# adeebkor/fenicsx-fus

Measured on AMD Instinct MI355X. Metric: DOF-updates/sec (RK4 step) at p=4 hex fp64, higher is better.
Workload: dtype f64; 1 GPU; 3D homogeneous wave, hex p=4 f64, Linear RK4, weak scaling: 64^3 cells per GPU (BASELINE.json configs[1]); ndofs_global=16974593, cells_per_gpu=262144, medium=water, partition=x-slabs x1, transport=none, blocks=8192, mfma_contractions=False, mfma_4x4x4_index1=False, packed_fp32=False, lds_bytes_per_block=72504

## Files before the change

### fenicsx-fus_amd/csrc/fusmi.hip

```cpp
#include "../../include/fusmi.h"

#include <dlfcn.h>
#include <hip/hip_runtime.h>
#include <rccl/rccl.h>
#include <limits>

#include <algorithm>
#include <cmath>
#include <cstdio>
#include <cstring>
#include <atomic>
#include <map>
#include <mutex>
#include <tuple>
#include <memory>
#include <string>
#include <vector>

#include "kernels.hpp"
#include "layout.hpp"
#include "tables.hpp"

using namespace fus;

// ... 131 lines not shown

struct fus_op
{
  fus_ctx* ctx;
  int P, N, Nd, dtype;
  int tdim = 3;
  size_t ts;
  int64_t ncells, ndofs, nnodes;
  Layout L;
  std::vector<double> nodes, wts, D;
  std::vector<char> h_geom_x;
  std::vector<int32_t> h_geom_dm;
  int geom_order = 1, geom_nv = 8;
  std::vector<int32_t> h_dofmap;
  BlockArgs A{};
  std::vector<void*> allocs;
  int32_t *d_cell_perm = nullptr, *d_dof_perm = nullptr;
  int64_t *d_sh_ptr = nullptr, *d_sh_pairs = nullptr;
  void *d_G = nullptr, *d_detJ = nullptr, *d_Dg = nullptr, *d_partial = nullptr;
  void *d_tmp_x = nullptr, *d_tmp_b = nullptr, *d_tmp_c = nullptr, *d_tmp_coef = nullptr;
  size_t lds_bytes = 0;
  int deterministic = 0;
  int nfields = 1;
  bool affine = false;
  bool trilinear = false;
  bool mfma = false;
  bool ortho_mesh = false;
  bool diag = false;
  bool pk = false;
  void* d_Gc = nullptr;
// ... 8 lines not shown

struct fus_model
{
  fus_ctx* ctx;
  fus_op* op;
  int kind;
  hipGraphExec_t gexec = nullptr;
  int64_t gsteps = 0;
  double freq, amp, speed;
  void *u0 = nullptr, *v0 = nullptr, *u_ = nullptr, *v_ = nullptr, *un = nullptr, *vn = nullptr,
       *b = nullptr, *minv = nullptr, *m = nullptr, *coef = nullptr, *coef2 = nullptr;
  void* d_bsrc2 = nullptr;
  void* mn1 = nullptr;
  int64_t nb = 0, nb_int = 0;
  int32_t* d_bidx = nullptr;
  int32_t* d_blk_bnd_off = nullptr;
  int32_t *d_sh_ptr32 = nullptr, *d_sh_pairs32 = nullptr;
  uint64_t* d_bnd_mask = nullptr;
  int32_t* d_bnd_base = nullptr;
  void *d_bsrc = nullptr, *d_babs = nullptr;
  std::vector<void*> allocs;
  bool initialised = false;
  bool setup_done = false;
  int rk_order = 4;
  int forms = 0;
  int lean_rk4 = 1;
  bool bnd_valid = false;
  double bnd_tn = 0.0;
  int64_t rc_n = 0;
  int32_t* d_rc_idx = nullptr;
  void *d_rc_bas = nullptr, *d_rc_out = nullptr, *d_rec = nullptr;
// ... 65 lines not shown
};

template <typename T, int P, int OP, int ATOMIC, int STAGE, int NF, int GEOM, int TD = 3, int MF = 0, int PK = 0>
static int launch_block_op_v(fus_op* op, const T* geo, const T* coef, const T* x, T* bvec,
                             const StageArgs<T>& S, int blk_begin, int blk_count)
{
  if (blk_count <= 0)
    return FUS_OK;
  constexpr int N = P + 1;
  KArgs<T, N> K;
  for (int i = 0; i < N * N; ++i)
    K.Dk.d[i] = (T)op->D[i], K.Dk.dt[i] = (T)op->D[(i % N) * N + i / N];

  for (int i = 0; i < N; ++i)
    K.Dk.w[i] = (T)op->wts[i], K.Dk.x[i] = (T)op->nodes[i];
  static std::atomic<uint64_t> attr_set{0};
  const uint64_t dev_bit = 1ull << (op->ctx->device & 63);
  if (!(attr_set.load(std::memory_order_relaxed) & dev_bit))
  {
    HIPCHK(hipFuncSetAttribute(reinterpret_cast<const void*>(&k_block_op<T, P, OP, ATOMIC, STAGE, NF, GEOM, TD, MF, PK>),
                               hipFuncAttributeMaxDynamicSharedMemorySize, 160 * 1024));
    attr_set.fetch_or(dev_bit, std::memory_order_relaxed);
  }
  K.A = op->A;
  if (GEOM == GEOM_DIAG)
  {
    for (int q = 0; q < N; ++q)
      for (int i = 0; i < N; ++i)
      {
        double acc = 0;
        for (int m = 0; m < N; ++m)
          acc += op->D[m * N + q] * op->wts[m] * op->D[m * N + i];
        K.Dk.d[q * N + i] = K.Dk.dt[q * N + i] = (T)acc;
      }
  }
  K.A.blk_begin = blk_begin;
  K.A.blk_count = blk_count;
  K.Dg = static_cast<const T*>(op->d_Dg), K.geo = geo, K.coef = coef, K.x = x, K.bvec = bvec;
  K.partial = static_cast<T*>(op->d_partial);
  K.S = S;
  int grid = blk_count;
  if (GEOM != GEOM_STREAM && TD == 3 && op->ctx->walk != 0)
  {
    int per_cu = op->ctx->walk;
    if (per_cu < 0)
    {
      static std::mutex occ_mu;
      static std::map<std::tuple<int, int, size_t>, int> occ_cache;
      int occ = 0;
      {
        std::lock_guard<std::mutex> lk(occ_mu);
        const auto key = std::make_tuple(op->ctx->device, op->L.waves, op->lds_bytes);
        auto it = occ_cache.find(key);
        if (it == occ_cache.end())
        {
          int nb = 0;
          HIPCHK(hipOccupancyMaxActiveBlocksPerMultiprocessor(
              &nb, reinterpret_cast<const void*>(&k_block_op<T, P, OP, ATOMIC, STAGE, NF, GEOM, TD, MF, PK>), 64 * op->L.waves,
              op->lds_bytes));
          it = occ_cache.emplace(key, std::max(nb, 1)).first;
        }
        occ = it->second;
      }
      per_cu = (blk_count >= 4 * occ * op->ctx->num_cus) ? occ : 0;
    }
    if (per_cu > 0)
      grid = std::min(blk_count, per_cu * op->ctx->num_cus);
  }
  hipLaunchKernelGGL((k_block_op<T, P, OP, ATOMIC, STAGE, NF, GEOM, TD, MF, PK>), dim3(grid),
                     dim3(64 * op->L.waves), op->lds_bytes, op->ctx->stream, K);
  HIPCHK(hipGetLastError());
  return FUS_OK;
}

template <typename T, int P, int OP, int STAGE, int NF = 1>
static int launch_block_op(fus_op* op, const T* geo, const T* coef, const T* x, T* bvec,
                           const StageArgs<T>& S, int blk_begin = 0, int blk_count = -1)
{
  if (NF > op->nfields)
    return fail(FUS_ERR_STATE, "operator data was not created for two-field models (option fields=2)");
  if (blk_count < 0)
    blk_count = op->L.nblocks - blk_begin;
  const int b0 = blk_begin, nb = blk_count;
  if constexpr (P >= 8)
// ... 225 lines not shown
static bool mfma_default(int P, bool f64, bool affine)
{
  (void)P, (void)f64, (void)affine;
  return false;
}

template <typename T, int P>
static int op_setup_device(fus_op* op)
{
  constexpr int N = P + 1;
  fus_ctx* c = op->ctx;
  hipStream_t st = c->stream;
  Layout& L = op->L;
  auto& pool = op->allocs;

  std::vector<ShapeDev> shapes(L.shapes.size());
  for (size_t i = 0; i < shapes.size(); ++i)
  {
    shapes[i].nelem = L.shapes[i].nelem, shapes[i].nloc = L.shapes[i].nloc;
    shapes[i].nint = L.shapes[i].nint, shapes[i].nrounds = L.shapes[i].nrounds;
    shapes[i].rounds_off = L.shapes[i].rounds_off, shapes[i].ldm_off = L.shapes[i].ldm_off;
  }
  int32_t *d_blk_shape, *d_elem_off, *d_int_off, *d_sh_gidx;
  int64_t* d_sh_off;
  ShapeDev* d_shapes;
  int16_t* d_rounds;
  uint16_t* d_ldm;
  FUSCHK(upload(pool, &d_blk_shape, L.blk_shape, st));
  FUSCHK(upload(pool, &d_shapes, shapes, st));
  FUSCHK(upload(pool, &d_elem_off, L.blk_elem_off, st));
  FUSCHK(upload(pool, &d_int_off, L.blk_int_off, st));
  FUSCHK(upload(pool, &d_sh_off, L.blk_sh_off, st));
  FUSCHK(upload(pool, &d_sh_gidx, L.sh_gidx, st));
  FUSCHK(upload(pool, &d_rounds, L.rounds, st));
  L.ldm.resize((L.ldm.size() + 15) & ~(size_t)15);
  FUSCHK(upload(pool, &d_ldm, L.ldm, st));
  FUSCHK(upload(pool, &op->d_cell_perm, L.cell_perm, st));
  FUSCHK(upload(pool, &op->d_dof_perm, L.dof_perm, st));
  FUSCHK(upload(pool, &op->d_sh_ptr, L.sh_ptr, st));
  {
    std::vector<int64_t> pos(L.sh_pairs.size());
    for (size_t k = 0; k < pos.size(); ++k)
      pos[k] = L.pair_pos[L.sh_pairs[k]];
    FUSCHK(upload(pool, &op->d_sh_pairs, pos, st));
  }
  int32_t* d_sh_ppos;
  FUSCHK(upload(pool, &d_sh_ppos, L.pair_pos, st));
  op->A.sh_ppos = d_sh_ppos;
  op->A.blk_shape = d_blk_shape, op->A.shapes = d_shapes, op->A.blk_elem_off = d_elem_off;
  op->A.blk_int_off = d_int_off, op->A.blk_sh_off = d_sh_off, op->A.sh_gidx = d_sh_gidx;
  op->A.rounds = d_rounds, op->A.ldm = d_ldm, op->A.nblocks = L.nblocks;
  op->A.lds_nloc = (L.max_nloc + 1) & ~1;
  op->A.waves = L.waves;
  op->A.lds_nelem = (L.max_nelem + 7) & ~7;
  op->lds_bytes = L.lds_bytes(sizeof(T), op->nfields);
  if (op->lds_bytes > 160 * 1024)
    return fail(FUS_ERR_LIMIT, "block does not fit 160 KB of LDS; lower block_elems");

  std::vector<T> Dg(N * N + 2 * N);
  for (int i = 0; i < N * N; ++i)
    Dg[i] = (T)op->D[i];
  for (int i = 0; i < N; ++i)
    Dg[N * N + i] = (T)op->wts[i], Dg[N * N + N + i] = (T)op->nodes[i];
  T* d_Dg;
  FUSCHK(upload(pool, &d_Dg, Dg, st));
// ... 326 lines not shown
      bidx.push_back((int32_t)i);
      bsrc.push_back(src[i]);
      babs.push_back(absb[i]);
      if (lossy)
        bsrc2.push_back(src2[i]);
    }
  m->nb = (int64_t)bidx.size();
  {
    const Layout& L = op->L;
    m->nb_int = std::lower_bound(bidx.begin(), bidx.end(), (int32_t)L.n_int_pad) - bidx.begin();
    std::vector<int32_t> off(L.nblocks + 1);
    for (int32_t b = 0; b < L.nblocks; ++b)
      off[b] = (int32_t)(std::lower_bound(bidx.begin(), bidx.begin() + m->nb_int, L.blk_int_off[b])
                         - bidx.begin());
    off[L.nblocks] = (int32_t)m->nb_int;
    FUSCHK(upload(m->allocs, &m->d_blk_bnd_off, off, st));
    if (L.n_partial + L.n_shared > 2000000000ll)
      return fail(FUS_ERR_LIMIT, "partial slab exceeds int32 indexing");
    std::vector<int32_t> extra(L.n_shared, -1);
    for (int64_t k = m->nb_int; k < m->nb; ++k)
      extra[bidx[k] - L.n_int_pad] = (int32_t)(L.n_partial + (k - m->nb_int));
    std::vector<int32_t> ptr(L.n_shared + 1), prs;
    prs.reserve(L.npairs + (m->nb - m->nb_int));
    for (int64_t sidx = 0; sidx < L.n_shared; ++sidx)
    {
      ptr[sidx] = (int32_t)prs.size();
      for (int64_t k = L.sh_ptr[sidx]; k < L.sh_ptr[sidx + 1]; ++k)
        prs.push_back(L.pair_pos[L.sh_pairs[k]]);
      if (extra[sidx] >= 0)
        prs.push_back(extra[sidx]);
    }
// ... 126 lines not shown
  default: return {C, B, A};
  }
}

template <typename T>
static StageArgs<T> stage_args(fus_model* m, int i, const StageScalars& sc)
{
  StageArgs<T> S;
  const StageVel<T> V = stage_vel<T>(m, i);
  S.minv = static_cast<const T*>(m->minv);
  S.vn = V.vn, S.un = static_cast<T*>(m->un);
  S.u0 = static_cast<T*>(m->u0), S.v0 = static_cast<T*>(m->v0);
  S.u_ = V.u_, S.v_ = V.v_;
  S.adt = (T)sc.adt, S.bdt = (T)sc.bdt, S.gval = (T)sc.gval;
  S.b0dt = (T)sc.b0dt, S.pdt = (T)sc.pdt, S.third = T(1) / T(3);
  S.blk_bnd_off = m->d_blk_bnd_off, S.bnd_idx = m->d_bidx;
  S.bnd_src = static_cast<const T*>(m->d_bsrc), S.bnd_abs = static_cast<const T*>(m->d_babs);
  S.x2 = nullptr, S.coef2 = static_cast<const T*>(m->coef2);
  S.bnd_src2 = static_cast<const T*>(m->d_bsrc2), S.dgval = (T)sc.dgval;
  S.m0 = static_cast<const T*>(m->m), S.mn1 = static_cast<const T*>(m->mn1);
  return S;
}

template <typename T, int P>
static int stage_begin(fus_model* m, int i, double t, double dt)
{
  fus_op* op = m->op;
  const T* ustage = static_cast<const T*>(i == 0 ? m->u0 : m->un);
  T* b = static_cast<T*>(m->b);
  StageArgs<T> S = stage_args<T>(m, i, stage_scalars<T>(m, i, t, dt));
  const T* vstage = i == 0 ? static_cast<const T*>(m->v0) : S.vn;
// ... 1750 lines not shown
  if (op->dtype == FUS_F64)
    hipLaunchKernelGGL((k_from_internal<double, 0>), dim3(nblk(op->ndofs)), dim3(256), 0, st,
                       op->ndofs, op->d_dof_perm, static_cast<const double*>(m->m),
                       static_cast<double*>(op->d_tmp_c));
  else
    hipLaunchKernelGGL((k_from_internal<float, 0>), dim3(nblk(op->ndofs)), dim3(256), 0, st,
                       op->ndofs, op->d_dof_perm, static_cast<const float*>(m->m),
                       static_cast<float*>(op->d_tmp_c));
  HIPCHK(hipMemcpyAsync(out, op->d_tmp_c, op->ndofs * op->ts, hipMemcpyDeviceToHost, st));
  HIPCHK(hipStreamSynchronize(st));
  return FUS_OK;
}

int64_t fus_model_ndofs(fus_model* m) { return m ? m->op->ndofs : 0; }

int fus_measure_bandwidth(fus_ctx* c, int64_t nbytes, int reps, double* gbps)
{
  if (!c || !gbps || nbytes < (1 << 20) || reps < 1)
    return fail(FUS_ERR_ARG, "bad argument");
  HIPCHK(hipSetDevice(c->device));
  typedef double D2 __attribute__((ext_vector_type(2)));
  const int64_t nvec = nbytes / 16;
  D2 *x = nullptr, *y = nullptr;
  HIPCHK(hipMalloc(&x, nvec * 16));
  HIPCHK(hipMalloc(&y, nvec * 16));
  HIPCHK(hipMemsetAsync(x, 0, nvec * 16, c->stream));
  HIPCHK(hipMemsetAsync(y, 0, nvec * 16, c->stream));
  hipEvent_t e0, e1;
  HIPCHK(hipEventCreate(&e0));
  HIPCHK(hipEventCreate(&e1));
// ... 76 lines not shown
```

### fenicsx-fus_amd/csrc/kernels.hpp

```cpp
#pragma once
#include <hip/hip_runtime.h>
#include <stdint.h>

#include "geom.hpp"

namespace fus
{

struct ShapeDev
{
  int32_t nelem, nloc, nint, nrounds;
  int64_t rounds_off, ldm_off;
};

struct BlockArgs
{
  const int32_t* blk_shape;
  const ShapeDev* shapes;
  const int32_t* blk_elem_off;
  const int32_t* blk_int_off;
  const int64_t* blk_sh_off;
  const int32_t* sh_gidx;
  const int32_t* sh_ppos;
  const int16_t* rounds;
  const uint16_t* ldm;
  int32_t nblocks;
  int32_t blk_begin;
  int32_t blk_count;
  int32_t lds_nloc;
  int32_t lds_nelem;
  int32_t waves;
};

template <typename T>
struct StageArgs
{
  const T* minv;
  T *vn, *un, *u0, *v0, *u_, *v_;
  T adt, bdt, gval;
  T b0dt, pdt, third;
  const int32_t* blk_bnd_off;
  const int32_t* bnd_idx;
  const T* bnd_src;
  const T* bnd_abs;
  const T* x2;
  const T* coef2;
  const T* bnd_src2;
  T dgval;
  const T* m0;
  const T* mn1;
};

enum
{
  STAGE_NONE = -1
};
// ... 113 lines not shown
    return 1;
  if (P == 5)
    return (sizeof(T) == 4 && geom == GEOM_TRILINEAR) ? FUS_EPIU : 1;
  if (sizeof(T) == 4 && P == 7)
    return geom == GEOM_TRILINEAR ? FUS_EPIU + 2 : FUS_EPIU_F32P7AFF;
  if (sizeof(T) == 8 && P == 6 && is_aff(geom))
    return 1;
  return FUS_EPIU;
}
template <typename T>
__host__ __device__ constexpr bool epi_early(int P)
{
  return sizeof(T) == 8 && P <= 5;
}

__host__ __device__ constexpr int geom_cell_stride(int geom)
{
  return is_aff(geom) ? 7 : (geom == GEOM_TRILINEAR ? 21 : 0);
}

__device__ __forceinline__ double fast_rcp(double x)
{
  double r = __builtin_amdgcn_rcp(x);
  r = __builtin_fma(__builtin_fma(-x, r, 1.0), r, r);
  r = __builtin_fma(__builtin_fma(-x, r, 1.0), r, r);
  return r;
}
__device__ __forceinline__ float fast_rcp(float x)
{
  float r = __builtin_amdgcn_rcpf(x);
// ... 1825 lines not shown
  const T* geo;
  const T* coef;
  const T* x;
  T* bvec;
  T* partial;
  StageArgs<T> S;
};

template <typename T, int N>
__device__ __forceinline__ void load_stage_args(const KArgs<T, N> __attribute__((address_space(4))) * q, StageArgs<T>& S)
{
  S.minv = q->S.minv;
  S.vn = q->S.vn, S.un = q->S.un, S.u0 = q->S.u0, S.v0 = q->S.v0, S.u_ = q->S.u_, S.v_ = q->S.v_;
  S.adt = q->S.adt, S.bdt = q->S.bdt, S.gval = q->S.gval;
  S.b0dt = q->S.b0dt, S.pdt = q->S.pdt, S.third = q->S.third;
  S.blk_bnd_off = q->S.blk_bnd_off, S.bnd_idx = q->S.bnd_idx;
  S.bnd_src = q->S.bnd_src, S.bnd_abs = q->S.bnd_abs;
  S.x2 = q->S.x2, S.coef2 = q->S.coef2, S.bnd_src2 = q->S.bnd_src2, S.dgval = q->S.dgval;
  S.m0 = q->S.m0, S.mn1 = q->S.mn1;
}

template <typename T, int P, int OP, int ATOMIC, int STAGE, int NF, int GEOM, int TD = 3, int MF = 0, int PK = 0>
__global__ void __launch_bounds__((P <= 4) ? 512 : FUS_MID_THREADS, (P >= 8) ? FUS_HI_WAVES : (P <= 4 && is_aff(GEOM))
                                                            ? 4
                                                            : ((GEOM == GEOM_TRILINEAR || (is_aff(GEOM) && P <= 6)) ? FUS_TRI_WAVES_T(T, P) : (FUS_PF1(T, P, OP, ATOMIC, GEOM, TD) ? 2 : 1)))
k_block_op(const KArgs<T, P + 1> kernel_args)
{
  (void)kernel_args;
  static_assert(TD == 3 || GEOM == GEOM_STREAM, "quadrilaterals use the streamed geometry");
  typedef KArgs<T, P + 1> KArgsT;
  typedef DTab<T, P + 1> DTabT;
  static_assert(offsetof(KArgsT, Dk) == sizeof(BlockArgs) && offsetof(DTabT, dt) == sizeof(T) * ((P + 1) * (P + 1) + 2 * (P + 1)),
                "dtab_row reads the table at these kernarg offsets");
  constexpr int N = P + 1, N2 = N * N, Nd = (TD == 3) ? N * N * N : N * N;
  constexpr int EPW = (64 / N2) > 0 ? (64 / N2) : 1;
  constexpr int LPE = (N2 <= 64) ? 64 : 128;
  constexpr int SLOT = tile_slot_entries<T, N, TD>();
  static_assert(N2 <= 128, "degrees up to 10");
  static_assert(LPE == 64 || !MF, "degrees 8-10: no matrix-core variants");
  static_assert(!PK || (sizeof(T) == 4 && EPW == 1 && LPE == 64 && TD == 3 && OP == OP_STIFFNESS && ATOMIC && !MF
                        && GEOM != GEOM_STREAM),
                "packed path: fp32 stiffness, degrees 5-7, per-cell geometry, LDS-atomic accumulation");
  constexpr int EPS = PK ? 2 : 1;

  typedef const KArgs<T, N> __attribute__((address_space(4))) * KP;
#define FUS_KARGS(q)                                                                               \
  KP q = (KP)__builtin_amdgcn_kernarg_segment_ptr();                             \
  asm volatile("" : "+s"(q))
  constexpr int GCS = geom_cell_stride(GEOM);
  constexpr int AW = 8 / (int)sizeof(T);
  typedef double A2 __attribute__((ext_vector_type(2)));
  extern __shared__ __align__(16) unsigned char smem_raw[];
#define FUS_PHASE_LDS(q)                                                                           \
  const int lds_nloc = q->A.lds_nloc, lds_nelem = q->A.lds_nelem, nwaves = q->A.waves;             \
  const int slots = (nwaves * 64 / LPE) * EPW * EPS;                                               \
  T* x_l = reinterpret_cast<T*>(smem_raw);                                                         \
  double* y_l = reinterpret_cast<double*>(x_l + lds_nloc);  \
  T* x2_l = reinterpret_cast<T*>(y_l + lds_nloc);                 \
// ... 18 lines not shown
  const int lane = tid % LPE, wave = tid / LPE;         \
  const int s = lane / N2, p = lane - s * N2;                                                      \
  const int b = p / N, c = p - b * N;                                                              \
  const bool active = s < EPW;                                                                     \
  const int myslot = (wave * EPW + (active ? s : 0)) * EPS;                                        \
                                \
  T* sA = reinterpret_cast<T*>(smem_raw) + (size_t)((NF == 2 ? 2 : 1) + AW) * q->A.lds_nloc         \
          + (size_t)myslot * SLOT;                                                                 \
  T* sB = sA

  struct Meta
  {
    ShapeDev sh;
    int elem_off, int_off;
    int64_t sh_off;
  };
  auto meta_of = [&](KP q, int bk) -> Meta
  {
    Meta M;
    M.sh = q->A.shapes[q->A.blk_shape[bk]];
    M.elem_off = q->A.blk_elem_off[bk];
    M.int_off = q->A.blk_int_off[bk];
    M.sh_off = q->A.blk_sh_off[bk];
    return M;
  };
  typedef T V2 __attribute__((ext_vector_type(2)));
  typedef uint32_t U4 __attribute__((ext_vector_type(4)));
  constexpr int UI = (P <= 3) ? 3 : ((P == 4) ? 2 : (P <= 6 ? 4 : (P == 7 ? FUS_UI_P7 : FUS_UI_HI))),
                US = (P <= 3) ? 4 : ((P == 4) ? 3 : (P <= 7 ? 5 : FUS_UI_HI)),
                UL = (P <= 3) ? 2 : ((P == 4) ? 1 : 4);
  struct PLoad
  {
    V2 xi[UI], xi2[UI];
    T xs[US], xs2[US];
    U4 lq[UL];
    T cfv, cf2v, gcv, gcv2, dgv, xtail, xtail2;
  };
  auto p_idx = [&](KP q, const Meta& M, bool enable, int (&gi)[US]) __attribute__((always_inline))
  {
    FUS_TID();
    const int nsh = M.sh.nloc - M.sh.nint;
    const int32_t* gix = q->A.sh_gidx + M.sh_off;
#pragma unroll
    for (int u = 0; u < US; ++u)
      gi[u] = (enable && tid + u * nthr < nsh) ? gix[tid + u * nthr] : -1;
  };
  auto p_load = [&](KP q, const Meta& M, PLoad& L, bool with_tables, bool enable, const int (&gi)[US])
      __attribute__((always_inline))
  {
    FUS_TID();
    const ShapeDev& sh = M.sh;
    const T* __restrict__ x = q->x;
    const T* __restrict__ x2 = (NF == 2) ? q->S.x2 : x;
    const T* __restrict__ coef = q->coef;
    const T* __restrict__ coef2 = (NF == 2) ? q->S.coef2 : coef;
    const T* __restrict__ geo = q->geo;
    const T* __restrict__ Dg = q->Dg;
    const V2* xg = reinterpret_cast<const V2*>(x + M.int_off);
    const V2* xg2 = reinterpret_cast<const V2*>(x2 + M.int_off);
    const int nvec = sh.nint >> 1;
    const int nsh = sh.nloc - sh.nint;
    const int32_t* gix = q->A.sh_gidx + M.sh_off;
    const int n16 = (sh.nelem * Nd * 2 + 15) >> 4;
    const U4* lsrc = reinterpret_cast<const U4*>(q->A.ldm + sh.ldm_off);
    const int ngc = sh.nelem * GCS;
#pragma unroll
    for (int u = 0; u < UI; ++u)
    {
      const bool ok = enable && tid + u * nthr < nvec;
      L.xi[u] = ok ? xg[tid + u * nthr] : V2(T(0));
      L.xi2[u] = (NF == 2 && ok) ? xg2[tid + u * nthr] : V2(T(0));
    }
#pragma unroll
    for (int u = 0; u < UL; ++u)
      L.lq[u] = (enable && tid + u * nthr < n16) ? lsrc[tid + u * nthr] : U4(0u);
    L.cfv = (enable && tid < sh.nelem) ? coef[M.elem_off + tid] : T(0);
    L.cf2v = (NF == 2 && enable && tid < sh.nelem) ? coef2[M.elem_off + tid] : T(0);
    L.gcv = (enable && tid < ngc) ? geo[(int64_t)M.elem_off * GCS + tid] : T(0);
    L.gcv2 = (GCS > 7 && enable && tid + nthr < ngc) ? geo[(int64_t)M.elem_off * GCS + tid + nthr] : T(0);
    L.dgv = (with_tables && enable && tid < N2 + 2 * N) ? Dg[tid] : T(0);
// ... 163 lines not shown
  int blk = wg + q0->A.blk_begin;
  FUS_STAMP(blk, 0);
  ElemIn<T, N, OP, GEOM, TD> inA, inB;
  auto first_fetch = [&](KP q, const Meta& Mm) __attribute__((always_inline))
  {
    FUS_LANE_COORDS(q);
    (void)b, (void)c, (void)sA, (void)sB;
    const int slots = (q->A.waves * 64 / LPE) * EPW * EPS;
    const int nt0 = ATOMIC ? (Mm.sh.nelem + slots - 1) / slots : Mm.sh.nrounds;
    int e0 = -1;
    if (active && nt0 > 0)
      e0 = ATOMIC ? (myslot < Mm.sh.nelem ? myslot : -1) : (int)q->A.rounds[Mm.sh.rounds_off + myslot];
    elem_fetch<T, N, OP, GEOM, TD>(inA, e0, q->geo, Mm.elem_off, p);
  };
  PLoad L;
  {
    const Meta M0 = meta_of(q0, blk);
    first_fetch(q0, M0);
    int gi0[US];
    p_idx(q0, M0, true, gi0);
    p_load(q0, M0, L, true, true, gi0);
  }
  bool first = true;
  for (;;)
  {
  FUS_KARGS(qc);
  FUS_PHASE_LDS(qc);
  FUS_LANE_COORDS(qc);
  const Meta M = meta_of(qc, blk);
  const ShapeDev& sh = M.sh;
  const int elem_off = M.elem_off;
  const int ntrips = ATOMIC ? (sh.nelem + slots - 1) / slots : sh.nrounds;
  auto elem_of = [&](int r) -> int
  {
    if (!active || r >= ntrips)
      return -1;
    if (ATOMIC)
      return (r * slots + myslot < sh.nelem) ? r * slots + myslot : -1;
    return (int)rt_l[r * slots + myslot];
  };
#ifdef FUS_PROBE_PFREE
  if (first)
    p_commit(qc, M, L, true);
  else
  {
    FUS_TID();
    for (int i = tid; i < (M.sh.nloc + 1) / 2; i += nthr)
      reinterpret_cast<A2*>(y_l)[i] = A2(0.0);
  }
#else
  p_commit(qc, M, L, first);
#endif
  const int blk_next = blk + blk_stride;
  const bool has_next = blk_next < blk_end;
  constexpr bool IDX_EARLY = false;
  int gi_n[US];
  if constexpr (IDX_EARLY)
  {
    Meta Mi{};
    if (has_next)
      Mi = meta_of(qc, blk_next);
    p_idx(qc, Mi, has_next, gi_n);
  }
  __syncthreads();
  FUS_STAMP(blk, 1);
#ifdef FUS_STAGGER
  if (tid0 >= 256)
    __builtin_amdgcn_s_sleep(FUS_STAGGER);
#endif
// ... 6 lines not shown
      constexpr bool inreg = (OP == OP_STIFFNESS) && !(FUS_PF1(T, P, OP, ATOMIC, GEOM, TD) && P >= 6)
                             && GEOM != GEOM_TRILINEAR && GEOM != GEOM_DIAG && !(is_aff(GEOM) && (P == 5 || P == 6)) && !MF;
      Drb[j] = inreg ? D_l[b * N + j] : T(0);
      Drc[j] = inreg ? D_l[c * N + j] : T(0);
      Dcb[j] = inreg ? D_l[j * N + b] : T(0);
      Dcc[j] = inreg ? D_l[j * N + c] : T(0);
    }
#pragma unroll
    for (int a = 0; a < N; ++a)
      w3[a] = (GEOM == GEOM_AFFINE) ? w_l[a] * w_l[b] * w_l[c] : T(0);
    wbc = (GEOM == GEOM_TRILINEAR || GEOM == GEOM_DIAG) ? w_l[b] * w_l[c] : T(0);
    pb = (GEOM == GEOM_TRILINEAR) ? pt_l[b] : T(0), pc = (GEOM == GEOM_TRILINEAR) ? pt_l[c] : T(0);
  }

  FUS_KARGS(qt);
  DTab<T, N> Dk;
  if constexpr (!dtab_by_rows<T, N>())
  {
#pragma unroll
    for (int i = 0; i < N * N; ++i)
      Dk.d[i] = qt->Dk.d[i];
  }
#pragma unroll
  for (int i = 0; i < N; ++i)
    Dk.w[i] = qt->Dk.w[i], Dk.x[i] = qt->Dk.x[i];
  const T* __restrict__ geo = qt->geo;
#define FUS_ELEM_COMPUTE(in)                                                                       \
  do                                                                                               \
  {                                                                                                \
    if constexpr (LPE == 128 && TD == 2)                                                           \
      elem_compute2d<T, N, OP, ATOMIC, NF, true>(in, Drb, Drc, Dcb, Dcc, x_l, y_l, sA, ldm_l,      \
                                                 cf_l, x2_l, cf2_l, p, b, c, s == 0);              \
    else if constexpr (LPE == 128)                                                                 \
      elem_compute_hi<T, N, OP, ATOMIC, NF, GEOM>(in.er, s == 0, Dk, x_l, y_l, sA, ldm_l, cf_l,    \
                                                  x2_l, cf2_l, gc_l, D_l, w_l, pt_l, p, b, c, geo, \
                                                  elem_off);                                       \
    else if constexpr (MF && TD == 3 && OP == OP_STIFFNESS)                                        \
      elem_compute_mfma<T, N, ATOMIC, NF, GEOM>(in, Dk, x_l, y_l, sA, ldm_l, cf_l, x2_l, cf2_l,    \
                                                gc_l, w3, D_l, wbc, pb, pc, p, lane);              \
    else if constexpr (TD == 3)                                                                    \
// ... 53 lines not shown
    }
  }
#undef FUS_ELEM_COMPUTE
  {
  FUS_KARGS(qe);
  FUS_PHASE_LDS(qe);
  FUS_TID();
  const Meta M = meta_of(qe, blk);
  const ShapeDev& sh = M.sh;
  const int int_off = M.int_off;
  const int64_t sh_off = M.sh_off;
  StageArgs<T> S;
  load_stage_args<T, N>(qe, S);
  T* __restrict__ bvec = qe->bvec;
  T* __restrict__ partial = qe->partial;
  const int32_t* __restrict__ pp = qe->A.sh_ppos + sh_off;
  const int nsh = sh.nloc - sh.nint;
  int ppv[US];
#pragma unroll
  for (int u = 0; u < US; ++u)
    ppv[u] = (tid + u * nthr < nsh) ? pp[tid + u * nthr] : -1;

  const int nvec = sh.nint >> 1;
    constexpr bool EPI2 = (P <= 4) && (NF == 1);
    struct Epi
    {
      bool on;
      int i, o;
      V2 bv, mi, w, a0, b0, au, av, m1, m0v, us;
    };
    auto epi_load = [&](int i, Epi& E, int part) __attribute__((always_inline))
    {
      if (part != 2)
      {
      E.on = i < nvec;
      E.i = i, E.o = int_off + 2 * i;
      E.bv = E.mi = E.w = E.a0 = E.b0 = E.au = E.av = E.m1 = E.m0v = E.us = V2(T(0));
#ifdef FUS_PROBE_EFREE
      auto ld = [&](const T* ptr) -> V2 { return E.on ? V2(T(1)) + V2(T((uintptr_t)ptr & 7)) : V2(T(0)); };
#else
      auto ld = [&](const T* ptr) -> V2
      { return E.on ? __builtin_nontemporal_load(reinterpret_cast<const V2*>(ptr + E.o)) : V2(T(0)); };
#endif
      constexpr bool WV = NF == 2;
      if (STAGE == 0)
        E.a0 = ld(S.u0), E.b0 = ld(S.v0);
      else if (STAGE == 4)
        E.b0 = ld(S.v0);
      else
        E.w = ld(S.vn);
      if (WV && S.mn1)
        E.m1 = ld(S.mn1), E.m0v = ld(S.m0);
      else
        E.mi = ld(S.minv);
      if (STAGE == 3)
        E.au = ld(S.u_), E.av = ld(S.v_);
      else if (STAGE == 1)
// ... 67 lines not shown
        st(S.vn, kv * S.adt + E.b0);
      }
    };
    constexpr int EPIU = EPI2 ? 2 : epiu_of<T>(P, GEOM, NF);
    constexpr bool EARLY = epi_early<T>(P);
    Epi Ef[EPIU];
    if (EARLY && STAGE != STAGE_NONE)
    {
#pragma unroll
      for (int u = 0; u < EPIU; ++u)
        epi_load(tid + u * nthr, Ef[u], 1);
    }
  __syncthreads();
  FUS_STAMP(blk, 2);

  {
    FUS_KARGS(qn);
    Meta Mn{};
    if (has_next)
      Mn = meta_of(qn, blk_next);
#ifdef FUS_PROBE_PFREE
    if constexpr (!IDX_EARLY)
      p_idx(qn, Mn, false, gi_n);
    p_load(qn, Mn, L, false, false, gi_n);
#else
    if constexpr (!IDX_EARLY)
      p_idx(qn, Mn, has_next, gi_n);
    p_load(qn, Mn, L, false, has_next, gi_n);
#endif
  }
  if (STAGE == STAGE_NONE)
  {
    V2* bg = reinterpret_cast<V2*>(bvec + int_off);
    for (int i = tid; i < nvec; i += nthr)
    {
      const A2 a2 = reinterpret_cast<const A2*>(y_l)[i];
      bg[i] = V2{(T)a2[0], (T)a2[1]};
    }
    if (tid == 0 && (sh.nint & 1))
      bvec[int_off + sh.nint - 1] = (T)y_l[sh.nint - 1];
  }
  else
  {
    const int k0 = S.blk_bnd_off[blk], k1 = S.blk_bnd_off[blk + 1];
    if (k1 > k0)
    {
      const T* vstage = stage_is_first(STAGE) ? S.v0 : S.vn;
      for (int k = k0 + tid; k < k1; k += nthr)
      {
        const int gi = S.bnd_idx[k];
        T add = S.gval * S.bnd_src[k] - S.bnd_abs[k] * vstage[gi];
        if (NF == 2)
          add += S.dgval * S.bnd_src2[k];
        y_l[gi - int_off] += add;
      }
      __syncthreads();
    }
    if (tid == 0 && (sh.nint & 1))
      (void)stage_update_dof<T, STAGE>((int64_t)int_off + sh.nint - 1, (T)y_l[sh.nint - 1], S.minv, S.vn, S.un, S.u0,
// ... 12 lines not shown
      for (int u = 0; u < EPIU; ++u)
        epi_load(i + u * nthr, E[u], 0);
#pragma unroll
      for (int u = 0; u < EPIU; ++u)
        epi_store(E[u]);
    }
  }
#pragma unroll
  for (int u = 0; u < US; ++u)
    if (ppv[u] >= 0)
      partial[ppv[u]] = (T)y_l[sh.nint + tid + u * nthr];
  for (int k = tid + US * nthr; k < nsh; k += nthr)
    partial[pp[k]] = (T)y_l[sh.nint + k];
  }
  FUS_TRACE_END(blk);
  if (!has_next)
    break;
  __syncthreads();
  blk = blk_next;
  first = false;
  {
    FUS_KARGS(qf);
    const Meta Mf = meta_of(qf, blk);
    first_fetch(qf, Mf);
  }
  }
#undef FUS_KARGS
#undef FUS_LANE_COORDS
#undef FUS_PHASE_LDS
#undef FUS_TID
}
// ... 513 lines not shown
```

### fenicsx-fus_amd/fenicsxfus_amd/_abi.py

```python
from __future__ import annotations

import ctypes as C
import os

import numpy as np

_HERE = os.path.dirname(os.path.abspath(__file__))
LIB_PATH = os.environ.get("FUSMI_LIB", os.path.join(_HERE, "libfusmi.so"))

FUS_F32, FUS_F64 = 0, 1
FUS_HOST, FUS_DEVICE = 0, 1
FUS_LINEAR, FUS_LOSSY, FUS_WESTERVELT = 0, 1, 2
FUS_U, FUS_V = 0, 1
FUS_MON_MAX, FUS_MON_MIN, FUS_MON_MEAN, FUS_MON_RMS, FUS_MON_COS, FUS_MON_SIN = range(6)

SYMBOLS = [
    "fus_last_error", "fus_version", "fus_init", "fus_finalize", "fus_synchronize", "fus_set_option",
    "fus_comm_unique_id", "fus_comm_init", "fus_comm_selftest", "fus_op_create", "fus_op_destroy", "fus_stiffness_apply",
    "fus_mass_apply", "fus_op_get_geometry", "fus_op_get_tables", "fus_op_info", "fus_op_is_affine", "fus_op_geometry_mode", "fus_op_uses_mfma", "fus_op_uses_diag_metric", "fus_op_uses_mfma4", "fus_op_uses_pack32", "fus_op_hmin", "fus_op_norm2", "fus_comm_allreduce", "fus_facet_diag",
    "fus_op_set_neighbours", "fus_model_create", "fus_model_destroy", "fus_model_set_rk_order", "fus_model_init", "fus_model_rk4",
    "fus_model_rk4_steps", "fus_model_get", "fus_model_set", "fus_model_get_mass", "fus_model_ndofs",
    "fus_profile_enable", "fus_profile_get", "fus_measure_bandwidth", "fus_layout_check", "fus_layout_check_ex", "fus_comm_init_local",
    "fus_group_finish_setup", "fus_group_rk4_steps", "fus_op_halo_layout", "fus_op_halo_buffers",
    "fus_model_setup_count", "fus_model_setup_pack", "fus_model_setup_unpack", "fus_model_setup_finish",
    "fus_model_stage_begin", "fus_model_stage_end",
    "fus_model_set_receivers", "fus_model_sample", "fus_model_record", "fus_model_get_records",
    "fus_model_monitor", "fus_model_monitor_get", "fus_model_monitor_info",
]


class FusError(RuntimeError):
    pass


_lib = None

# ... 134 lines not shown
```

### fenicsx-fus_amd/fenicsxfus_amd/models.py

```python
from __future__ import annotations

import ctypes as C

import numpy as np

from . import _abi
from ._abi import Context, check, lib, ptr
from .mesh import Function, FunctionSpace
from .operators import SpectralOperatorData, _array


class _SpectralExplicit:

    _kind = _abi.FUS_LINEAR

    def _create(self, mesh, meshtags, k, c0, rho0, delta0, freq0, p0, s0, rk_order, dt, V, ctx, beta0=None,
                forms="cpp"):
        if rk_order not in (1, 2, 3, 4):
            raise _abi.FusError("rk_order must be 1, 2, 3 or 4 (_linear.py:286-311)")
        if forms not in ("cpp", "python"):
            raise _abi.FusError("forms must be 'cpp' or 'python'")
        self.mesh, self.dt = mesh, dt
        self.freq, self.p0, self.s0 = float(freq0), float(p0), float(s0)
        self.V = V or FunctionSpace(mesh, k)
# ... 143 lines not shown
                                          ptr(f.x.array), C.c_int(_abi.FUS_HOST)))
        return f

    def u_sol(self):
        self._pull()
        return self.u_n

    def number_of_dofs(self):
        return self.V.dofmap.index_map.size_global

    def mass_vector(self):
        out = np.empty(self.data.ndofs, dtype=self.data.dtype)
        check(lib().fus_model_get_mass(self.h, ptr(out)))
        return out

    def close(self):
        if self.h:
            lib().fus_model_destroy(self.h)
            self.h = C.c_void_p()
        self.data.close()


class LinearSpectralExplicit(_SpectralExplicit):

    _kind = _abi.FUS_LINEAR

    def __init__(self, mesh, meshtags, k, c0, rho0, freq0, p0, s0, rk_order=4, dt=None, V=None,
                 ctx: Context | None = None):
        self._create(mesh, meshtags, k, c0, rho0, None, freq0, p0, s0, rk_order, dt, V, ctx)

# ... 33 lines not shown
```

### include/fusmi.h

```cpp
#ifndef FUSMI_H
#define FUSMI_H

#include <stdint.h>

#ifdef __cplusplus
extern "C" {
#endif

#define FUS_OK 0
#define FUS_ERR_ARG (-1)
#define FUS_ERR_HIP (-2)
#define FUS_ERR_RCCL (-3)
#define FUS_ERR_STATE (-4)
#define FUS_ERR_LIMIT (-5)

enum { FUS_F32 = 0, FUS_F64 = 1 };
enum { FUS_HOST = 0, FUS_DEVICE = 1 };
enum { FUS_LINEAR = 0, FUS_LOSSY = 1, FUS_WESTERVELT = 2 };
enum { FUS_U = 0, FUS_V = 1 };

typedef struct fus_ctx fus_ctx;
typedef struct fus_op fus_op;
typedef struct fus_model fus_model;

// ... 43 lines not shown

int fus_model_create(fus_ctx* ctx, int kind, fus_op* op, const void* c0, const void* rho0,
                     const void* delta0, const void* beta0, int64_t nfacets,
                     const int32_t* facet_cells, const int32_t* facet_local,
                     const int32_t* facet_tags, double freq, double amp, double speed,
                     fus_model** model);
int fus_model_destroy(fus_model* model);
int fus_model_set_rk_order(fus_model* model, int order);
int fus_model_init(fus_model* model);
int fus_model_rk4(fus_model* model, double t0, double tf, double dt, int64_t* nsteps);
int fus_model_rk4_steps(fus_model* model, double t0, double dt, int64_t nsteps);
int fus_model_get(fus_model* model, int which, void* out, int space);
int fus_model_set(fus_model* model, int which, const void* in, int space);
int fus_model_get_mass(fus_model* model, void* out);
int64_t fus_model_ndofs(fus_model* model);

int fus_model_set_receivers(fus_model* model, int64_t npts, const int32_t* cells, const double* refcoords);
int fus_model_sample(fus_model* model, int which, void* out, int space);
int fus_model_record(fus_model* model, int which, int every, int64_t capacity);
int fus_model_get_records(fus_model* model, void* out, double* times, int64_t* nrec);

enum { FUS_MON_MAX = 0, FUS_MON_MIN = 1, FUS_MON_MEAN = 2, FUS_MON_RMS = 3, FUS_MON_COS = 4, FUS_MON_SIN = 5 };
int fus_model_monitor(fus_model* model, int which, int nharm, double freq, int64_t skip, int every, int64_t count);
int fus_model_monitor_get(fus_model* model, int quantity, int k, void* out, int space);
int fus_model_monitor_info(fus_model* model, int64_t* nsamples, double* t_first, double* t_last);

int fus_group_finish_setup(fus_model** models, int n);
int fus_group_rk4_steps(fus_model** models, int n, double t0, double dt, int64_t nsteps);

int fus_op_halo_layout(fus_op* op, int* nneigh, int32_t* ranks, int64_t* counts, int64_t* offsets);
// ... 24 lines not shown
```

Measured before the change: 13.93 billion DOF-updates/s.

## Pack per-block metadata into 64-byte descriptors and specialise non-walking kernel

Per-block layout metadata (shape, element, interior and shared offsets, boundary range), previously spread across several arrays with an indirect shape lookup, is merged into one 64-byte descriptor that can be read as a single scalar load. The block kernel gains a WALK template parameter. The non-walking variant drops the next-block prefetch loop, loads the D tables early into scalar registers, and uses branch-free clamped loads in place of predicated ones. The aim is to cut scalar-memory latency and divergent control flow at block start, at the cost of one more kernel instantiation and redundant clamped loads. A block_info diagnostic API is also added.

```diff
diff --git a/fenicsx-fus_amd/csrc/fusmi.hip b/fenicsx-fus_amd/csrc/fusmi.hip
--- a/fenicsx-fus_amd/csrc/fusmi.hip
+++ b/fenicsx-fus_amd/csrc/fusmi.hip
@@ -169,6 +169,7 @@
   int geom_order = 1, geom_nv = 8;
   std::vector<int32_t> h_dofmap;
   BlockArgs A{};
+  std::vector<BlockDesc> h_desc;
   std::vector<void*> allocs;
   int32_t *d_cell_perm = nullptr, *d_dof_perm = nullptr;
   int64_t *d_sh_ptr = nullptr, *d_sh_pairs = nullptr;
@@ -207,7 +208,8 @@
   void* mn1 = nullptr;
   int64_t nb = 0, nb_int = 0;
   int32_t* d_bidx = nullptr;
-  int32_t* d_blk_bnd_off = nullptr;
+  BlockDesc* d_blk_desc = nullptr;
+  std::vector<int32_t> h_blk_bnd_off;
   int32_t *d_sh_ptr32 = nullptr, *d_sh_pairs32 = nullptr;
   uint64_t* d_bnd_mask = nullptr;
   int32_t* d_bnd_base = nullptr;
@@ -303,12 +305,16 @@
 
   for (int i = 0; i < N; ++i)
     K.Dk.w[i] = (T)op->wts[i], K.Dk.x[i] = (T)op->nodes[i];
+  constexpr bool CAN_WALK = GEOM != GEOM_STREAM && TD == 3;
   static std::atomic<uint64_t> attr_set{0};
   const uint64_t dev_bit = 1ull << (op->ctx->device & 63);
   if (!(attr_set.load(std::memory_order_relaxed) & dev_bit))
   {
-    HIPCHK(hipFuncSetAttribute(reinterpret_cast<const void*>(&k_block_op<T, P, OP, ATOMIC, STAGE, NF, GEOM, TD, MF, PK>),
+    HIPCHK(hipFuncSetAttribute(reinterpret_cast<const void*>(&k_block_op<T, P, OP, ATOMIC, STAGE, NF, GEOM, TD, MF, PK, 0>),
                                hipFuncAttributeMaxDynamicSharedMemorySize, 160 * 1024));
+    if constexpr (CAN_WALK)
+      HIPCHK(hipFuncSetAttribute(reinterpret_cast<const void*>(&k_block_op<T, P, OP, ATOMIC, STAGE, NF, GEOM, TD, MF, PK, 1>),
+                                 hipFuncAttributeMaxDynamicSharedMemorySize, 160 * 1024));
     attr_set.fetch_or(dev_bit, std::memory_order_relaxed);
   }
   K.A = op->A;
@@ -329,7 +335,8 @@
   K.partial = static_cast<T*>(op->d_partial);
   K.S = S;
   int grid = blk_count;
-  if (GEOM != GEOM_STREAM && TD == 3 && op->ctx->walk != 0)
+  bool walking = false;
+  if (CAN_WALK && op->ctx->walk != 0)
   {
     int per_cu = op->ctx->walk;
     if (per_cu < 0)
@@ -345,7 +352,7 @@
         {
           int nb = 0;
           HIPCHK(hipOccupancyMaxActiveBlocksPerMultiprocessor(
-              &nb, reinterpret_cast<const void*>(&k_block_op<T, P, OP, ATOMIC, STAGE, NF, GEOM, TD, MF, PK>), 64 * op->L.waves,
+              &nb, reinterpret_cast<const void*>(&k_block_op<T, P, OP, ATOMIC, STAGE, NF, GEOM, TD, MF, PK, CAN_WALK ? 1 : 0>), 64 * op->L.waves,
               op->lds_bytes));
           it = occ_cache.emplace(key, std::max(nb, 1)).first;
         }
@@ -354,9 +361,19 @@
       per_cu = (blk_count >= 4 * occ * op->ctx->num_cus) ? occ : 0;
     }
     if (per_cu > 0)
-      grid = std::min(blk_count, per_cu * op->ctx->num_cus);
-  }
-  hipLaunchKernelGGL((k_block_op<T, P, OP, ATOMIC, STAGE, NF, GEOM, TD, MF, PK>), dim3(grid),
+      grid = std::min(blk_count, per_cu * op->ctx->num_cus), walking = true;
+  }
+  if constexpr (CAN_WALK)
+  {
+    if (walking)
+    {
+      hipLaunchKernelGGL((k_block_op<T, P, OP, ATOMIC, STAGE, NF, GEOM, TD, MF, PK, 1>), dim3(grid), dim3(64 * op->L.waves),
+                         op->lds_bytes, op->ctx->stream, K);
+      HIPCHK(hipGetLastError());
+      return FUS_OK;
+    }
+  }
+  hipLaunchKernelGGL((k_block_op<T, P, OP, ATOMIC, STAGE, NF, GEOM, TD, MF, PK, 0>), dim3(grid),
                      dim3(64 * op->L.waves), op->lds_bytes, op->ctx->stream, K);
   HIPCHK(hipGetLastError());
   return FUS_OK;
@@ -612,23 +629,20 @@
   Layout& L = op->L;
   auto& pool = op->allocs;
 
-  std::vector<ShapeDev> shapes(L.shapes.size());
-  for (size_t i = 0; i < shapes.size(); ++i)
-  {
-    shapes[i].nelem = L.shapes[i].nelem, shapes[i].nloc = L.shapes[i].nloc;
-    shapes[i].nint = L.shapes[i].nint, shapes[i].nrounds = L.shapes[i].nrounds;
-    shapes[i].rounds_off = L.shapes[i].rounds_off, shapes[i].ldm_off = L.shapes[i].ldm_off;
-  }
-  int32_t *d_blk_shape, *d_elem_off, *d_int_off, *d_sh_gidx;
-  int64_t* d_sh_off;
-  ShapeDev* d_shapes;
+  op->h_desc.assign(L.nblocks, BlockDesc{});
+  for (int32_t b = 0; b < L.nblocks; ++b)
+  {
+    const Layout::Shape& hs = L.shapes[L.blk_shape[b]];
+    BlockDesc& d = op->h_desc[b];
+    d.sh.nelem = hs.nelem, d.sh.nloc = hs.nloc, d.sh.nint = hs.nint, d.sh.nrounds = hs.nrounds;
+    d.sh.rounds_off = hs.rounds_off, d.sh.ldm_off = hs.ldm_off;
+    d.elem_off = L.blk_elem_off[b], d.int_off = L.blk_int_off[b], d.sh_off = L.blk_sh_off[b];
+  }
+  int32_t* d_sh_gidx;
+  BlockDesc* d_desc;
   int16_t* d_rounds;
   uint16_t* d_ldm;
-  FUSCHK(upload(pool, &d_blk_shape, L.blk_shape, st));
-  FUSCHK(upload(pool, &d_shapes, shapes, st));
-  FUSCHK(upload(pool, &d_elem_off, L.blk_elem_off, st));
-  FUSCHK(upload(pool, &d_int_off, L.blk_int_off, st));
-  FUSCHK(upload(pool, &d_sh_off, L.blk_sh_off, st));
+  FUSCHK(upload(pool, &d_desc, op->h_desc, st));
   FUSCHK(upload(pool, &d_sh_gidx, L.sh_gidx, st));
   FUSCHK(upload(pool, &d_rounds, L.rounds, st));
   L.ldm.resize((L.ldm.size() + 15) & ~(size_t)15);
@@ -645,8 +659,7 @@
   int32_t* d_sh_ppos;
   FUSCHK(upload(pool, &d_sh_ppos, L.pair_pos, st));
   op->A.sh_ppos = d_sh_ppos;
-  op->A.blk_shape = d_blk_shape, op->A.shapes = d_shapes, op->A.blk_elem_off = d_elem_off;
-  op->A.blk_int_off = d_int_off, op->A.blk_sh_off = d_sh_off, op->A.sh_gidx = d_sh_gidx;
+  op->A.desc = d_desc, op->A.sh_gidx = d_sh_gidx;
   op->A.rounds = d_rounds, op->A.ldm = d_ldm, op->A.nblocks = L.nblocks;
   op->A.lds_nloc = (L.max_nloc + 1) & ~1;
   op->A.waves = L.waves;
@@ -1003,7 +1016,11 @@
       off[b] = (int32_t)(std::lower_bound(bidx.begin(), bidx.begin() + m->nb_int, L.blk_int_off[b])
                          - bidx.begin());
     off[L.nblocks] = (int32_t)m->nb_int;
-    FUSCHK(upload(m->allocs, &m->d_blk_bnd_off, off, st));
+    std::vector<BlockDesc> desc(op->h_desc);
+    for (int32_t b = 0; b < L.nblocks; ++b)
+      desc[b].bnd0 = off[b], desc[b].bnd1 = off[b + 1];
+    FUSCHK(upload(m->allocs, &m->d_blk_desc, desc, st));
+    m->h_blk_bnd_off = off;
     if (L.n_partial + L.n_shared > 2000000000ll)
       return fail(FUS_ERR_LIMIT, "partial slab exceeds int32 indexing");
     std::vector<int32_t> extra(L.n_shared, -1);
@@ -1160,7 +1177,7 @@
   S.u_ = V.u_, S.v_ = V.v_;
   S.adt = (T)sc.adt, S.bdt = (T)sc.bdt, S.gval = (T)sc.gval;
   S.b0dt = (T)sc.b0dt, S.pdt = (T)sc.pdt, S.third = T(1) / T(3);
-  S.blk_bnd_off = m->d_blk_bnd_off, S.bnd_idx = m->d_bidx;
+  S.blk_desc = m->d_blk_desc, S.bnd_idx = m->d_bidx;
   S.bnd_src = static_cast<const T*>(m->d_bsrc), S.bnd_abs = static_cast<const T*>(m->d_babs);
   S.x2 = nullptr, S.coef2 = static_cast<const T*>(m->coef2);
   S.bnd_src2 = static_cast<const T*>(m->d_bsrc2), S.dgval = (T)sc.dgval;
@@ -2941,6 +2958,29 @@
 
 int64_t fus_model_ndofs(fus_model* m) { return m ? m->op->ndofs : 0; }
 
+int fus_model_block_info(fus_model* m, int64_t out[8])
+{
+  if (!m || !out)
+    return fail(FUS_ERR_ARG, "null argument");
+  if (!m->setup_done)
+    return fail(FUS_ERR_STATE, "model setup has not finished");
+  const Layout& L = m->op->L;
+  for (int i = 0; i < 8; ++i)
+    out[i] = 0;
+  out[0] = L.nblocks;
+  out[2] = out[4] = INT64_MAX;
+  for (int32_t b = 0; b < L.nblocks; ++b)
+  {
+    const Layout::Shape& sh = L.shapes[L.blk_shape[b]];
+    const int64_t nint = sh.nint, nsh = sh.nloc - sh.nint;
+    out[1] += nint & 1;
+    out[2] = std::min(out[2], nint), out[3] = std::max(out[3], nint);
+    out[4] = std::min(out[4], nsh), out[5] = std::max(out[5], nsh);
+    out[m->h_blk_bnd_off[b + 1] > m->h_blk_bnd_off[b] ? 6 : 7] += 1;
+  }
+  return FUS_OK;
+}
+
 int fus_measure_bandwidth(fus_ctx* c, int64_t nbytes, int reps, double* gbps)
 {
   if (!c || !gbps || nbytes < (1 << 20) || reps < 1)
diff --git a/fenicsx-fus_amd/csrc/kernels.hpp b/fenicsx-fus_amd/csrc/kernels.hpp
--- a/fenicsx-fus_amd/csrc/kernels.hpp
+++ b/fenicsx-fus_amd/csrc/kernels.hpp
@@ -13,13 +13,19 @@
   int64_t rounds_off, ldm_off;
 };
 
+struct BlockDesc
+{
+  ShapeDev sh;
+  int32_t elem_off, int_off;
+  int64_t sh_off;
+  int32_t bnd0, bnd1;
+  int32_t pad[2];
+};
+static_assert(sizeof(BlockDesc) == 64, "one s_load_dwordx16 per block");
+
 struct BlockArgs
 {
-  const int32_t* blk_shape;
-  const ShapeDev* shapes;
-  const int32_t* blk_elem_off;
-  const int32_t* blk_int_off;
-  const int64_t* blk_sh_off;
+  const BlockDesc* desc;
   const int32_t* sh_gidx;
   const int32_t* sh_ppos;
   const int16_t* rounds;
@@ -39,7 +45,7 @@
   T *vn, *un, *u0, *v0, *u_, *v_;
   T adt, bdt, gval;
   T b0dt, pdt, third;
-  const int32_t* blk_bnd_off;
+  const BlockDesc* blk_desc;
   const int32_t* bnd_idx;
   const T* bnd_src;
   const T* bnd_abs;
@@ -183,6 +189,14 @@
   return sizeof(T) == 8 && P <= 5;
 }
 
+template <typename T>
+__host__ __device__ constexpr bool block_branch_free(int P, int geom, int walk)
+{
+  if (sizeof(T) == 4 && P == 5 && geom == GEOM_STREAM)
+    return false;
+  return !walk;
+}
+
 __host__ __device__ constexpr int geom_cell_stride(int geom)
 {
   return is_aff(geom) ? 7 : (geom == GEOM_TRILINEAR ? 21 : 0);
@@ -2038,13 +2052,13 @@
   S.vn = q->S.vn, S.un = q->S.un, S.u0 = q->S.u0, S.v0 = q->S.v0, S.u_ = q->S.u_, S.v_ = q->S.v_;
   S.adt = q->S.adt, S.bdt = q->S.bdt, S.gval = q->S.gval;
   S.b0dt = q->S.b0dt, S.pdt = q->S.pdt, S.third = q->S.third;
-  S.blk_bnd_off = q->S.blk_bnd_off, S.bnd_idx = q->S.bnd_idx;
+  S.blk_desc = q->S.blk_desc, S.bnd_idx = q->S.bnd_idx;
   S.bnd_src = q->S.bnd_src, S.bnd_abs = q->S.bnd_abs;
   S.x2 = q->S.x2, S.coef2 = q->S.coef2, S.bnd_src2 = q->S.bnd_src2, S.dgval = q->S.dgval;
   S.m0 = q->S.m0, S.mn1 = q->S.mn1;
 }
 
-template <typename T, int P, int OP, int ATOMIC, int STAGE, int NF, int GEOM, int TD = 3, int MF = 0, int PK = 0>
+template <typename T, int P, int OP, int ATOMIC, int STAGE, int NF, int GEOM, int TD = 3, int MF = 0, int PK = 0, int WALK = 0>
 __global__ void __launch_bounds__((P <= 4) ? 512 : FUS_MID_THREADS, (P >= 8) ? FUS_HI_WAVES : (P <= 4 && is_aff(GEOM))
                                                             ? 4
                                                             : ((GEOM == GEOM_TRILINEAR || (is_aff(GEOM) && P <= 6)) ? FUS_TRI_WAVES_T(T, P) : (FUS_PF1(T, P, OP, ATOMIC, GEOM, TD) ? 2 : 1)))
@@ -2066,6 +2080,8 @@
                         && GEOM != GEOM_STREAM),
                 "packed path: fp32 stiffness, degrees 5-7, per-cell geometry, LDS-atomic accumulation");
   constexpr int EPS = PK ? 2 : 1;
+  constexpr bool BF = block_branch_free<T>(P, GEOM, WALK);
+  constexpr bool DK_EARLY = !WALK && P <= 4;
 
   typedef const KArgs<T, N> __attribute__((address_space(4))) * KP;
 #define FUS_KARGS(q)                                                                               \
@@ -2114,14 +2130,18 @@
     ShapeDev sh;
     int elem_off, int_off;
     int64_t sh_off;
+    int bnd0, bnd1;
   };
   auto meta_of = [&](KP q, int bk) -> Meta
   {
+    typedef const BlockDesc __attribute__((address_space(4))) * DP;
+    const BlockDesc* g = (STAGE != STAGE_NONE) ? q->S.blk_desc : q->A.desc;
+    const DP d = (DP)(uintptr_t)g + bk;
     Meta M;
-    M.sh = q->A.shapes[q->A.blk_shape[bk]];
-    M.elem_off = q->A.blk_elem_off[bk];
-    M.int_off = q->A.blk_int_off[bk];
-    M.sh_off = q->A.blk_sh_off[bk];
+    M.sh.nelem = d->sh.nelem, M.sh.nloc = d->sh.nloc, M.sh.nint = d->sh.nint, M.sh.nrounds = d->sh.nrounds;
+    M.sh.rounds_off = d->sh.rounds_off, M.sh.ldm_off = d->sh.ldm_off;
+    M.elem_off = d->elem_off, M.int_off = d->int_off, M.sh_off = d->sh_off;
+    M.bnd0 = d->bnd0, M.bnd1 = d->bnd1;
     return M;
   };
   typedef T V2 __attribute__((ext_vector_type(2)));
@@ -2140,6 +2160,18 @@
   {
     FUS_TID();
     const int nsh = M.sh.nloc - M.sh.nint;
+    if constexpr (BF)
+    {
+      const int32_t* gix = q->A.sh_gidx + (nsh > 0 ? M.sh_off : (int64_t)0);
+#pragma unroll
+      for (int u = 0; u < US; ++u)
+      {
+        const bool ok = tid + u * nthr < nsh;
+        const int v = gix[ok ? tid + u * nthr : 0];
+        gi[u] = ok ? v : -1;
+      }
+      return;
+    }
     const int32_t* gix = q->A.sh_gidx + M.sh_off;
 #pragma unroll
     for (int u = 0; u < US; ++u)
@@ -2164,6 +2196,86 @@
     const int n16 = (sh.nelem * Nd * 2 + 15) >> 4;
     const U4* lsrc = reinterpret_cast<const U4*>(q->A.ldm + sh.ldm_off);
     const int ngc = sh.nelem * GCS;
+    if constexpr (BF)
+    {
+      const V2* xb = nvec > 0 ? xg : reinterpret_cast<const V2*>(x);
+      const V2* xb2 = nvec > 0 ? xg2 : reinterpret_cast<const V2*>(x2);
+#pragma unroll
+      for (int u = 0; u < UI; ++u)
+      {
+        const bool ok = tid + u * nthr < nvec;
+        const int i = ok ? tid + u * nthr : 0;
+        const V2 v = xb[i];
+        L.xi[u] = ok ? v : V2(T(0));
+        if constexpr (NF == 2)
+        {
+          const V2 v2 = xb2[i];
+          L.xi2[u] = ok ? v2 : V2(T(0));
+        }
+        else
+          L.xi2[u] = V2(T(0));
+      }
+#pragma unroll
+      for (int u = 0; u < UL; ++u)
+      {
+        const bool ok = tid + u * nthr < n16;
+        const U4 v = lsrc[ok ? tid + u * nthr : 0];
+        L.lq[u] = ok ? v : U4(0u);
+      }
+      {
+        const bool ok = tid < sh.nelem;
+        const T v = coef[M.elem_off + (ok ? tid : 0)];
+        L.cfv = ok ? v : T(0);
+        L.cf2v = T(0);
+        if constexpr (NF == 2)
+        {
+          const T v2 = coef2[M.elem_off + (ok ? tid : 0)];
+          L.cf2v = ok ? v2 : T(0);
+        }
+      }
+      L.gcv = L.gcv2 = T(0);
+      if constexpr (GCS > 0)
+      {
+        const bool ok = tid < ngc;
+        const T v = geo[(int64_t)M.elem_off * GCS + (ok ? tid : 0)];
+        L.gcv = ok ? v : T(0);
+      }
+      if constexpr (GCS > 7)
+      {
+        const bool ok = tid + nthr < ngc;
+        const T v = geo[(int64_t)M.elem_off * GCS + (ok ? tid + nthr : 0)];
+        L.gcv2 = ok ? v : T(0);
+      }
+      L.dgv = T(0);
+      if (with_tables)
+      {
+        const bool ok = tid < N2 + 2 * N;
+        const T v = Dg[ok ? tid : 0];
+        L.dgv = ok ? v : T(0);
+      }
+      {
+        const int64_t it = (sh.nint & 1) ? (int64_t)M.int_off + sh.nint - 1 : (int64_t)0;
+        L.xtail = x[it];
+        L.xtail2 = T(0);
+        if constexpr (NF == 2)
+          L.xtail2 = x2[it];
+      }
+#pragma unroll
+      for (int u = 0; u < US; ++u)
+      {
+        const bool ok = gi[u] >= 0;
+        const int g = ok ? gi[u] : 0;
+        const T v = x[g];
+        L.xs[u] = ok ? v : T(0);
+        L.xs2[u] = T(0);
+        if constexpr (NF == 2)
+        {
+          const T v2 = x2[g];
+          L.xs2[u] = ok ? v2 : T(0);
+        }
+      }
+      return;
+    }
 #pragma unroll
     for (int u = 0; u < UI; ++u)
     {
@@ -2357,20 +2469,33 @@
     elem_fetch<T, N, OP, GEOM, TD>(inA, e0, q->geo, Mm.elem_off, p);
   };
   PLoad L;
-  {
-    const Meta M0 = meta_of(q0, blk);
+  const Meta M0 = meta_of(q0, blk);
+  {
     first_fetch(q0, M0);
     int gi0[US];
     p_idx(q0, M0, true, gi0);
     p_load(q0, M0, L, true, true, gi0);
   }
+  DTab<T, N> Dk;
+  auto load_dk = [&](KP q) __attribute__((always_inline))
+  {
+    if constexpr (!dtab_by_rows<T, N>())
+    {
+#pragma unroll
+      for (int i = 0; i < N * N; ++i)
+        Dk.d[i] = q->Dk.d[i];
+    }
+#pragma unroll
+    for (int i = 0; i < N; ++i)
+      Dk.w[i] = q->Dk.w[i], Dk.x[i] = q->Dk.x[i];
+  };
   bool first = true;
   for (;;)
   {
   FUS_KARGS(qc);
   FUS_PHASE_LDS(qc);
   FUS_LANE_COORDS(qc);
-  const Meta M = meta_of(qc, blk);
+  const Meta M = WALK ? meta_of(qc, blk) : M0;
   const ShapeDev& sh = M.sh;
   const int elem_off = M.elem_off;
   const int ntrips = ATOMIC ? (sh.nelem + slots - 1) / slots : sh.nrounds;
@@ -2394,8 +2519,21 @@
 #else
   p_commit(qc, M, L, first);
 #endif
+  if constexpr (DK_EARLY)
+  {
+    load_dk(qc);
+#pragma unroll
+    for (int i = 0; i < N * N; ++i)
+      asm volatile("" : "+s"(Dk.d[i]));
+#pragma unroll
+    for (int i = 0; i < N; ++i)
+    {
+      asm volatile("" : "+s"(Dk.w[i]));
+      asm volatile("" : "+s"(Dk.x[i]));
+    }
+  }
   const int blk_next = blk + blk_stride;
-  const bool has_next = blk_next < blk_end;
+  const bool has_next = WALK && blk_next < blk_end;
   constexpr bool IDX_EARLY = false;
   int gi_n[US];
   if constexpr (IDX_EARLY)
@@ -2432,16 +2570,8 @@
   }
 
   FUS_KARGS(qt);
-  DTab<T, N> Dk;
-  if constexpr (!dtab_by_rows<T, N>())
-  {
-#pragma unroll
-    for (int i = 0; i < N * N; ++i)
-      Dk.d[i] = qt->Dk.d[i];
-  }
-#pragma unroll
-  for (int i = 0; i < N; ++i)
-    Dk.w[i] = qt->Dk.w[i], Dk.x[i] = qt->Dk.x[i];
+  if constexpr (!DK_EARLY)
+    load_dk(qt);
   const T* __restrict__ geo = qt->geo;
 #define FUS_ELEM_COMPUTE(in)                                                                       \
   do                                                                                               \
@@ -2525,12 +2655,21 @@
   load_stage_args<T, N>(qe, S);
   T* __restrict__ bvec = qe->bvec;
   T* __restrict__ partial = qe->partial;
-  const int32_t* __restrict__ pp = qe->A.sh_ppos + sh_off;
   const int nsh = sh.nloc - sh.nint;
+  const int32_t* __restrict__ pp = qe->A.sh_ppos + ((!BF || nsh > 0) ? sh_off : (int64_t)0);
   int ppv[US];
 #pragma unroll
   for (int u = 0; u < US; ++u)
-    ppv[u] = (tid + u * nthr < nsh) ? pp[tid + u * nthr] : -1;
+  {
+    if constexpr (BF)
+    {
+      const bool ok = tid + u * nthr < nsh;
+      const int v = pp[ok ? tid + u * nthr : 0];
+      ppv[u] = ok ? v : -1;
+    }
+    else
+      ppv[u] = (tid + u * nthr < nsh) ? pp[tid + u * nthr] : -1;
+  }
 
   const int nvec = sh.nint >> 1;
     constexpr bool EPI2 = (P <= 4) && (NF == 1);
@@ -2550,8 +2689,14 @@
 #ifdef FUS_PROBE_EFREE
       auto ld = [&](const T* ptr) -> V2 { return E.on ? V2(T(1)) + V2(T((uintptr_t)ptr & 7)) : V2(T(0)); };
 #else
+      const int lo = E.on ? E.o : (nvec > 0 ? int_off : 0);
       auto ld = [&](const T* ptr) -> V2
-      { return E.on ? __builtin_nontemporal_load(reinterpret_cast<const V2*>(ptr + E.o)) : V2(T(0)); };
+      {
+        if constexpr (BF)
+          return __builtin_nontemporal_load(reinterpret_cast<const V2*>(ptr + lo));
+        else
+          return E.on ? __builtin_nontemporal_load(reinterpret_cast<const V2*>(ptr + E.o)) : V2(T(0));
+      };
 #endif
       constexpr bool WV = NF == 2;
       if (STAGE == 0)
@@ -2649,6 +2794,7 @@
   __syncthreads();
   FUS_STAMP(blk, 2);
 
+  if constexpr (WALK)
   {
     FUS_KARGS(qn);
     Meta Mn{};
@@ -2677,7 +2823,7 @@
   }
   else
   {
-    const int k0 = S.blk_bnd_off[blk], k1 = S.blk_bnd_off[blk + 1];
+    const int k0 = M.bnd0, k1 = M.bnd1;
     if (k1 > k0)
     {
       const T* vstage = stage_is_first(STAGE) ? S.v0 : S.vn;
@@ -2720,7 +2866,7 @@
     partial[pp[k]] = (T)y_l[sh.nint + k];
   }
   FUS_TRACE_END(blk);
-  if (!has_next)
+  if (!WALK || !has_next)
     break;
   __syncthreads();
   blk = blk_next;
diff --git a/fenicsx-fus_amd/fenicsxfus_amd/_abi.py b/fenicsx-fus_amd/fenicsxfus_amd/_abi.py
--- a/fenicsx-fus_amd/fenicsxfus_amd/_abi.py
+++ b/fenicsx-fus_amd/fenicsxfus_amd/_abi.py
@@ -20,6 +20,7 @@
     "fus_mass_apply", "fus_op_get_geometry", "fus_op_get_tables", "fus_op_info", "fus_op_is_affine", "fus_op_geometry_mode", "fus_op_uses_mfma", "fus_op_uses_diag_metric", "fus_op_uses_mfma4", "fus_op_uses_pack32", "fus_op_hmin", "fus_op_norm2", "fus_comm_allreduce", "fus_facet_diag",
     "fus_op_set_neighbours", "fus_model_create", "fus_model_destroy", "fus_model_set_rk_order", "fus_model_init", "fus_model_rk4",
     "fus_model_rk4_steps", "fus_model_get", "fus_model_set", "fus_model_get_mass", "fus_model_ndofs",
+    "fus_model_block_info",
     "fus_profile_enable", "fus_profile_get", "fus_measure_bandwidth", "fus_layout_check", "fus_layout_check_ex", "fus_comm_init_local",
     "fus_group_finish_setup", "fus_group_rk4_steps", "fus_op_halo_layout", "fus_op_halo_buffers",
     "fus_model_setup_count", "fus_model_setup_pack", "fus_model_setup_unpack", "fus_model_setup_finish",
diff --git a/fenicsx-fus_amd/fenicsxfus_amd/models.py b/fenicsx-fus_amd/fenicsxfus_amd/models.py
--- a/fenicsx-fus_amd/fenicsxfus_amd/models.py
+++ b/fenicsx-fus_amd/fenicsxfus_amd/models.py
@@ -181,6 +181,13 @@
         check(lib().fus_model_get_mass(self.h, ptr(out)))
         return out
 
+    def block_info(self):
+        out = (C.c_int64 * 8)()
+        check(lib().fus_model_block_info(self.h, out))
+        keys = ["nblocks", "odd_interior_blocks", "min_interior", "max_interior", "min_shared", "max_shared",
+                "boundary_blocks", "plain_blocks"]
+        return dict(zip(keys, list(out)))
+
     def close(self):
         if self.h:
             lib().fus_model_destroy(self.h)
diff --git a/include/fusmi.h b/include/fusmi.h
--- a/include/fusmi.h
+++ b/include/fusmi.h
@@ -81,6 +81,7 @@
 int fus_model_set(fus_model* model, int which, const void* in, int space);
 int fus_model_get_mass(fus_model* model, void* out);
 int64_t fus_model_ndofs(fus_model* model);
+int fus_model_block_info(fus_model* model, int64_t out[8]);
 
 int fus_model_set_receivers(fus_model* model, int64_t npts, const int32_t* cells, const double* refcoords);
 int fus_model_sample(fus_model* model, int which, void* out, int space);
```

Result: faster. 15.62 billion DOF-updates/s, median of 6 (+12.2%).
